# mrinmoy-iitg/SM_HPSS_MTL

Hardware: AMD Instinct MI355X
Metric: clips/sec HPSS+MTL-CNN fwd (1s@16kHz) (higher is better)
Workload: dtype f32

## Files before the change

### sm_hpss_mtl_amd/csrc/smh_model.h

```cpp
#pragma once
#include "smh_common.h"

namespace smh_tcn {

using f32x4 = __attribute__((ext_vector_type(4))) float;

constexpr int C = 32;
constexpr int SX = 36;
constexpr int kMaxHeads = 4;
constexpr int kHidden = 16;
constexpr int kMaxG = 16;
constexpr int kPS = 80;
constexpr float kNormEps = 1e-5f;
constexpr float kBnEps = 1e-3f;
constexpr int kCat = kHidden + 2;
constexpr int kCatTail = 4 * kHidden + 4 * kCat + kCat + 1;
constexpr int kBlockFloats = 24 * 2 * 64 + 8 * 2 * 64 + 32 + 32;
constexpr size_t kNetLdsLimit = smh::kLdsBytesPerCU - 4 * 1024;

struct TcnArgs {
    int N, T, F, FQ, G, GRP, n_blocks, n_dil, vec_ok;
    int D, NH, n_mt, n_classes, n_heads, out_dim, skip_heads;
    int wlds;
    unsigned long long *trace;
    int tune;
    int *status;
    int spin_limit;
    int split_last;
    int from_x0;
    int x0_shift, x0_T;
    int head_odim[kMaxHeads];
    int head_sigmoid[kMaxHeads];
    int cascade;
    int single;
    int trunk_only;
    int x0_one;
    const float *pair_X, *pair_W0, *pair_Wb;
    float *pair_trunk;
    const float *pair_WhA, *pair_hp;
    float *pair_out;
    int *pair_status;
};

struct TrainIO {
    float *acts;
    const float *drop_tcn;
    float *pre;
    float *upre;
    int acts_last_only;
};

struct HeadsArgs {
    int N, D, NH, n_classes, n_heads, out_dim;
    int head_odim[kMaxHeads], head_sigmoid[kMaxHeads];
    float lw[kMaxHeads + 1];
    size_t goff_head[kMaxHeads];
    size_t goff_c3b;
    size_t hp_off[kMaxHeads];
    int ext_losses;
    int stamps;
};
struct HeadsPlan;
int launch_heads_train(const HeadsArgs &a, const HeadsPlan &p, const float *pre, const float *y, const float *hp, const float *drop,
                       float *dpre, float *dxh, float *grad, float *bnstat, float *losses, unsigned *ticket, hipStream_t st);
int launch_cascade_heads_train(const HeadsArgs &a, const HeadsPlan &p, const float *pre, const float *y, const float *hp,
                               const float *drop, float *dpre, float *dxh, float *dr, float *grad, float *bnstat, float *losses,
                               hipStream_t st);
// ... 21 lines not shown
    int *d_map = nullptr;
    size_t nW0, nWb, nWhA, nhp;
    void *d_bf16 = nullptr;
    unsigned long long version = 1, bf16_version = 0;
    int *d_status = nullptr;
};

namespace smh_tcn {
inline size_t head_tail_floats(const smh_model *m, int h) {
    const int od = m->head_odim[h], cat = m->head_cat[h];
    return cat ? (size_t)4 * kHidden + 4 * cat + (size_t)cat * od + od : (size_t)4 * kHidden + (size_t)kHidden * od + od;
}
struct Offsets {
    size_t w0_k, w0_b;
    size_t blk0, blk_stride;
    size_t c3_k, c3_b;
    size_t head[kMaxHeads];
    size_t trunk_p = 0;
    size_t fbn = 0;
};
inline size_t trunk_floats(const smh_model_cfg &c) {
    return (size_t)c.n_feat * C + C + (size_t)c.nb_stacks * c.n_dilations * (3 * C * C + C + C * C + C);
}
__host__ __device__ inline size_t v2_block0_floats(int F) {
    return (size_t)3 * F * C + C + 3 * C * C + C + (F != C ? (size_t)F * C + C : 0);
}
constexpr size_t kV2BlockFloats = 2 * (3 * C * C + C);
inline size_t trunk_floats_v2(const smh_model_cfg &c) {
    return v2_block0_floats(c.n_feat) + (size_t)(c.nb_stacks * c.n_dilations - 1) * kV2BlockFloats;
}
Offsets offsets(const smh_model *m);
struct ForwardSwitches {
    int G = 0, skew = -1, waves = 0;
    bool has_waves = false, prefetch = true, split = true, skew16 = false;
};
ForwardSwitches read_forward_switches();
struct ForwardPlan {
    int G, GRP, units, nwaves, mode, wlds, split_last;
    size_t lds;
};
int plan_forward(const smh_model *m, int N, bool train, bool trace, const ForwardSwitches &sw, ForwardPlan *p);
void fill_args(const smh_model *m, int N, const ForwardPlan &p, TcnArgs *a);
int dense_entry_ok(const char *name, const smh_model *m, const float *d_fv, int Tc, int shift, const void *d_work, size_t work_bytes,
                   size_t need_bytes, const float *d_out, int feat_multiple, const char *short_clip_entry);
int repack(smh_model *m, hipStream_t st);
int launch_forward_bf16_train(smh_model *m, const float *d_x, int N, const TrainIO *tio, hipStream_t st);
int forward_bf16_supported(const smh_model *m);
struct ForwardOpts {
    int from_x0 = 0, x0_shift = 0, x0_T = 0;
    int trunk_only = 0;
    int x0_one = 0;
    const smh_model *pair = nullptr;
    const float *pair_x = nullptr;
    float *pair_trunk = nullptr;
    float *pair_out = nullptr;
};
int launch_forward(const smh_model *m, const float *d_x, int N, float *d_out, float *d_trunk, const TrainIO *tio,
                   hipStream_t st, const ForwardOpts &opt = {});
int launch_l0_frames(const float *fv, const float *w0, float *x0, int rows, int Tc, hipStream_t st);
int launch_fusion_dense(const smh_model *m, int N, const float *xh, const float *xp, float *out, bool train, hipStream_t st);
size_t fusion_scratch_floats(const smh_model *m, int max_batch);
int launch_fusion_train(const smh_model *m, int N, int max_batch, const float *acts_h, const float *acts_p, float *scratch,
                        float *bnstat, float *pd, float *grad, int phase, hipStream_t st);
const float *fusion_gt(const smh_model *m, int max_batch, const float *scratch, int N, int b);
int launch_fusion_trunks(const smh_model *m, const float *xh, const float *xp, int N, float *tap_h, float *tap_p, ForwardOpts fo,
                         hipStream_t st);
// ... 3 lines not shown
```

### sm_hpss_mtl_amd/csrc/smh_tcn.hip

```cpp
#include <algorithm>
#include <cmath>
#include <cstdlib>
#include <cstring>
#include <type_traits>
#include <vector>

#include "smh_model.h"
#include "smh_tcn_heads.h"

using namespace smh_tcn;

namespace {

__device__ __forceinline__ f32x4 mfma4(float a, float b, f32x4 c) {
    return __builtin_amdgcn_mfma_f32_16x16x4f32(a, b, c, 0, 0, 0);
}

__device__ __forceinline__ float quad_max(float v) {
    const unsigned u = __float_as_uint(v);
    const auto r32 = __builtin_amdgcn_permlane32_swap(u, u, false, false);
    const float a = fmaxf(__uint_as_float(r32[0]), __uint_as_float(r32[1]));
    const unsigned ua = __float_as_uint(a);
    const auto r16 = __builtin_amdgcn_permlane16_swap(ua, ua, false, false);
    return fmaxf(__uint_as_float(r16[0]), __uint_as_float(r16[1]));
// ... 389 lines not shown
            }
        } else {
            for (int i = threadIdx.x; i < nW0; i += blockDim.x) w0s[i] = W0[i];
            __syncthreads();
            for (int u = wave; u < units; u += nw) {
                const int R = 16 * u + j;
                const int Rc = min(R, GR - 1);
                const float *xr = X + ((size_t)n0 * T + Rc) * a.F + (size_t)q * a.FQ;
                f32x4 c0 = bl, c1 = bh;
                for (int s = 0; s < a.FQ; ++s) {
                    const float xv = (q * a.FQ + s < a.F) ? xr[s] : 0.f;
                    c0 = mfma4(w0s[(s * 2 + 0) * 64 + lane], xv, c0);
                    c1 = mfma4(w0s[(s * 2 + 1) * 64 + lane], xv, c1);
                }
                float *dst = xa + (size_t)R * SX + 4 * q;
                *reinterpret_cast<f32x4 *>(dst) = c0;
                *reinterpret_cast<f32x4 *>(dst + 16) = c1;
            }
        }
    }

    float *ws = lds + 2 * (size_t)(a.GRP + 1) * SX;
    auto stage = [&](int blk) {
        const char *src = reinterpret_cast<const char *>(Wb + (size_t)blk * kBlockFloats);
        char *dst = reinterpret_cast<char *>(ws + (size_t)(blk & 1) * kBlockFloats);
        constexpr int nch = kBlockFloats * 4 / 16;
        for (int i = wave; i * 64 < nch; i += nw) {
            const int c = i * 64 + lane;
            if (c < nch)
                __builtin_amdgcn_global_load_lds((const __attribute__((address_space(1))) void *)(src + (size_t)c * 16),
                                                 (__attribute__((address_space(3))) void *)(dst + i * 1024), 16, 0, 0);
        }
    };
    TileInfo ti;
    ti.n = 0;
    const bool split = MODE == kPrefetch && a.split_last && units >= 2;
#pragma unroll
    for (int i = 0; i < kMaxTiles; ++i) {
        const int u = wave + i * nw;
        const int R = 16 * u + j, Rc = min(R, GR - 1);
        ti.R[i] = R, ti.g[i] = Rc / T, ti.t[i] = Rc - ti.g[i] * T;
        if (u < units - (split ? 1 : 0)) ti.n = i + 1;
    }
    {
        const int hw0 = (units - 1) % nw, hw1 = (hw0 + 1) % nw;
        ti.hrole = split ? (wave == hw0 ? 0 : (wave == hw1 ? 1 : -1)) : -1;
        const int R = 16 * (units - 1) + j, Rc = min(R, GR - 1);
        ti.hR = R, ti.hg = Rc / T, ti.ht = Rc - ti.hg * T;
    }
    float *xch = lds + 2 * (size_t)(a.GRP + 1) * SX + 2 * (size_t)kBlockFloats;
    if (split && threadIdx.x < 2) reinterpret_cast<int *>(xch + 2 * 64 * 4)[threadIdx.x] = 0;
    if (threadIdx.x < SX) xa[(size_t)ZR * SX + threadIdx.x] = 0.f, xb[(size_t)ZR * SX + threadIdx.x] = 0.f;
    float *xin = xa, *xout = xb;
    const int nslot = a.n_blocks + 1;
    auto save_acts = [&](const float *src, int slot) {
        if constexpr (TRAIN) {
            for (int i = threadIdx.x; i < GR * (C / 4); i += blockDim.x) {
                const int R = i >> 3, c4 = (i & 7) * 4;
                const int g = R / T, t = R - g * T;
                *reinterpret_cast<f32x4 *>(tio.acts + (((size_t)(n0 + g) * nslot + slot) * T + t) * C + c4) =
                    *reinterpret_cast<const f32x4 *>(src + (size_t)R * SX + c4);
            }
        }
    };
    const float *drop0 = TRAIN && tio.drop_tcn ? tio.drop_tcn + (size_t)n0 * a.n_blocks * C : nullptr;
    const int dstride = a.n_blocks * C;
// ... 5 lines not shown
                         ub0 ? ub0 + (size_t)blk * T * C : nullptr, ustride, prefetch, lane, xch, blk + 1, a.spin_limit, status);
        float *tmp = xin;
        xin = xout;
        xout = tmp;
    };
    if (MODE != kSkew && MODE != kSkew16 && tracing && blockIdx.x < 1024 && threadIdx.x == 0) {
        a.trace[4 * (2000 + blockIdx.x)] = __builtin_amdgcn_s_memtime();
        a.trace[4 * (2000 + blockIdx.x) + 1] = __builtin_amdgcn_s_memrealtime();
    }
    static_assert(!(TRAIN && MODE == kSkew16), "the 16-wave schedule is built for inference");
    float *flagbase = ws + (MODE == kSkew16 ? (size_t)kWeightRing * kBlockFloats : 0);
    if constexpr (MODE == kSkew || MODE == kSkew16) {
        typedef __attribute__((address_space(3))) volatile int lds_vint;
        lds_vint *done = (lds_vint *)(flagbase);
        if (threadIdx.x < 64) {
            int v = threadIdx.x == 62 ? nw : 0;
            if (MODE == kSkew16 && threadIdx.x >= 56 && threadIdx.x < 60)
                v = (threadIdx.x - 56 < 2 && threadIdx.x - 56 < a.n_blocks) ? threadIdx.x - 56 : -1;
            done[threadIdx.x] = v;
        }
        auto stage_ring = [&](int blk, int w0, int nwv) {
            const char *src = reinterpret_cast<const char *>(Wb + (size_t)blk * kBlockFloats);
            char *dst = reinterpret_cast<char *>(ws + (size_t)(blk & (kWeightRing - 1)) * kBlockFloats);
            constexpr int nch = kBlockFloats * 4 / 16;
            for (int i = w0; i * 64 < nch; i += nwv) {
                const int c = i * 64 + lane;
                if (c < nch)
                    __builtin_amdgcn_global_load_lds((const __attribute__((address_space(1))) void *)(src + (size_t)c * 16),
                                                     (__attribute__((address_space(3))) void *)(dst + i * 1024), 16, 0, 0);
            }
        };
        BlockW w0, w1;
        if constexpr (MODE == kSkew) {
            load_block_lds(w0, Wb, lane, q);
        } else {
            stage_ring(0, wave, nw);
            if (a.n_blocks > 1) stage_ring(1, wave, nw);
            asm volatile("s_waitcnt vmcnt(0)" ::: "memory");
        }
        __syncthreads();
        save_acts(xin, 0);
        if constexpr (TRAIN) __syncthreads();
        if (tracing && blockIdx.x < 1024 && threadIdx.x == 0) {
            a.trace[4 * (2000 + blockIdx.x)] = __builtin_amdgcn_s_memtime();
            a.trace[4 * (2000 + blockIdx.x) + 1] = __builtin_amdgcn_s_memrealtime();
        }
        const int n_tasks = a.n_blocks * units;
        const int m_units = (65536 + units - 1) / units, m_dil = (65536 + a.n_dil - 1) / a.n_dil;
        const unsigned m_T = (unsigned)(((1ull << 32) + (unsigned)T - 1) / (unsigned)T);
        const unsigned all_tiles = units >= 32 ? ~0u : (1u << units) - 1;
        const int xb_off = (a.GRP + 1) * SX, zrow = ZR * SX + 8 * q;
        struct Ops {
            f32x4 b[3][2], r0, r1;
            bool live0, live2;
            f32x4 dm0, dm1;
            int arow, urow;
        };
        auto dil = [&](int blk) { return 1 << (blk - ((blk * m_dil) >> 16) * a.n_dil); };
        auto ld4 = [&](int i) { return *reinterpret_cast<const f32x4 *>(__builtin_assume_aligned(lds + i, 16)); };
        auto issue_ops = [&](Ops &o, int blk, int u) {
            const int d = dil(blk);
            const int base = 16 * u, R = base + j;
            int g = (int)__umulhi((unsigned)base, m_T);
            int t = base - T * g + j;
            {
                const bool wr = t >= T;
// ... 213 lines not shown
                            if (stands(have, blk - 1, all_tiles)) break;
                            if (__any(lane == 63 && have != 0)) break;
                            if (spins > a.spin_limit) {
                                if (lane == 0) done[63] = 1;
                                break;
                            }
                            __builtin_amdgcn_s_sleep(1);
                        }
                    }
                    staged = blk + 2;
                    stage_ring(staged, 0, 1);
                }
                one_task(LdsWeights{ws + (size_t)(blk & (kWeightRing - 1)) * kBlockFloats, lane, q});
            }
        }
        publish();
        xin = (a.n_blocks & 1) ? xb : xa;
        xout = (a.n_blocks & 1) ? xa : xb;
        if (tracing && blockIdx.x < 1024 && threadIdx.x == 0) {
            a.trace[4 * (2000 + blockIdx.x) + 2] = __builtin_amdgcn_s_memtime();
            a.trace[4 * (2000 + blockIdx.x) + 3] = __builtin_amdgcn_s_memrealtime();
        }
    } else if (a.wlds && MODE == kPrefetch) {
        BlockW w0, w1;
        stage(0);
        if (a.n_blocks > 1) stage(1);
        asm volatile("s_waitcnt vmcnt(0)" ::: "memory");
        __syncthreads();
        load_block_lds(w0, ws, lane, q);
        for (int blk = 0; blk < a.n_blocks; blk += 2) {
            asm volatile("s_waitcnt vmcnt(0)" ::: "memory");
            __syncthreads();
            if (blk + 2 < a.n_blocks) stage(blk + 2);
            const bool more1 = blk + 1 < a.n_blocks;
            one_block(blk, w0, WeightPrefetch{w1, ws + kBlockFloats, lane, q});
            if (!more1) break;
            asm volatile("s_waitcnt vmcnt(0)" ::: "memory");
            __syncthreads();
            if (blk + 3 < a.n_blocks) stage(blk + 3);
            one_block(blk + 1, w1, WeightPrefetch{w0, ws, lane, q});
        }
    } else {
        if (a.wlds) stage(0);
        BlockW w;
        for (int blk = 0; blk < a.n_blocks; ++blk) {
            if (a.wlds) {
                asm volatile("s_waitcnt vmcnt(0)" ::: "memory");
                __syncthreads();
                if (blk + 1 < a.n_blocks) stage(blk + 1);
                one_block(blk, w, WeightLoad{w, ws + (size_t)(blk & 1) * kBlockFloats, lane, q});
            } else {
                __syncthreads();
                load_block_lds(w, Wb + (size_t)blk * kBlockFloats, lane, q);
                one_block(blk, w, NoPrefetch());
            }
        }
    }
    if (MODE != kSkew && MODE != kSkew16 && tracing && blockIdx.x < 1024 && threadIdx.x == 0) {
        a.trace[4 * (2000 + blockIdx.x) + 2] = __builtin_amdgcn_s_memtime();
        a.trace[4 * (2000 + blockIdx.x) + 3] = __builtin_amdgcn_s_memrealtime();
    }
    __syncthreads();
    if constexpr (MODE != kSkew && MODE != kSkew16) save_acts(xin, a.n_blocks);
    if constexpr (TRAIN) __syncthreads();
    for (int i = threadIdx.x; i < GR * (C / 4); i += blockDim.x) {
        const int R = i >> 3, c4 = (i & 7) * 4;
        f32x4 v = *reinterpret_cast<const f32x4 *>(xin + (size_t)R * SX + c4);
#pragma unroll
        for (int r = 0; r < 4; ++r) v[r] = fmaxf(v[r], 0.f);
        *reinterpret_cast<f32x4 *>(xin + (size_t)R * SX + c4) = v;
        if (trunk) *reinterpret_cast<f32x4 *>(trunk + ((size_t)n0 * T + R) * C + c4) = v;
    }
    __syncthreads();

    bool gave_up = false;
    if constexpr (MODE == kSkew || MODE == kSkew16) gave_up = ((__attribute__((address_space(3))) volatile int *)(flagbase))[63] != 0;
    dense_and_heads<TRAIN>(a, xin, xout, WhA, hp, out, tio, n0, g_here);
    if (tracing && blockIdx.x < 256 && threadIdx.x == 0) a.trace[4 * 3000 + 2 * blockIdx.x + 1] = __builtin_amdgcn_s_memrealtime();
    if (gave_up) {
        __syncthreads();
        for (int i = threadIdx.x; i < (a.trunk_only ? 0 : g_here * a.out_dim); i += blockDim.x) out[(size_t)n0 * a.out_dim + i] = 0.f;
        if (threadIdx.x == 0 && status) atomicOr(status, 1);
    }
}

__global__ void repack_kernel(const float *__restrict__ flat, const int *__restrict__ map, float *__restrict__ dst, size_t n) {
    const size_t i = (size_t)blockIdx.x * blockDim.x + threadIdx.x;
    if (i < n) {
        const int m = map[i];
        dst[i] = m ? flat[m - 1] : 0.f;
    }
}

static void pack_host(const smh_model *m, const float *h, std::vector<float> &W0, std::vector<float> &Wb,
                      std::vector<float> &WhA, std::vector<float> &hp) {
    const int F = m->cfg.n_feat, FQ = m->FQ, D = m->D, NH = m->NH, ncls = m->cfg.n_classes;
    W0.assign(m->nW0, 0.f), Wb.assign(m->nWb, 0.f), WhA.assign(m->nWhA, 0.f), hp.assign(m->nhp, 0.f);
    std::vector<float> Wh((size_t)D * NH, 0.f), bhv((size_t)m->n_mt * 16, 0.f);
    const float *p = h;
    if (m->heads == SMH_HEADS_FUSION) {
        p += 2 * trunk_floats(m->cfg) + (size_t)4 * D;
    } else if (m->cfg.block_variant == 1) {
        p += trunk_floats_v2(m->cfg);
    } else {
    for (int s = 0; s < FQ; ++s)
        for (int mt = 0; mt < 2; ++mt)
            for (int lane = 0; lane < 64; ++lane) {
                const int q = lane >> 4, i = lane & 15, f = q * FQ + s;
                W0[((size_t)s * 2 + mt) * 64 + lane] = f < F ? p[(size_t)f * C + 16 * mt + i] : 0.f;
            }
// ... 103 lines not shown
}

int repack(smh_model *m, hipStream_t st) {
    m->version++;
    if (m->heads == SMH_HEADS_FUSION) {
        const size_t tf = trunk_floats(m->cfg);
        for (int b = 0; b < 2; ++b) {
            SMH_CHECK_HIP(hipMemcpyAsync(m->trunk[b]->d_flat, m->d_flat + b * tf, tf * sizeof(float), hipMemcpyDeviceToDevice, st));
            const int rc = repack(m->trunk[b], st);
            if (rc) return rc;
            const size_t k0 = (size_t)m->cfg.n_feat * C;
            SMH_CHECK_HIP(hipMemcpyAsync(m->d_w0cat + b * k0, m->d_flat + b * tf, k0 * sizeof(float), hipMemcpyDeviceToDevice, st));
        }
    }
    const size_t n = m->nW0 + m->nWb + m->nWhA + m->nhp;
    hipLaunchKernelGGL(repack_kernel, dim3((unsigned)((n + 255) / 256)), dim3(256), 0, st, m->d_flat, m->d_map, m->d_W0, n);
    return smh::launch_status("repack_kernel");
}

void fill_args(const smh_model *m, int N, const ForwardPlan &p, TcnArgs *pa) {
    TcnArgs &a = *pa;
    a.N = N, a.T = m->cfg.patch_size, a.F = m->cfg.n_feat, a.FQ = m->FQ, a.n_blocks = m->n_blocks, a.n_dil = m->cfg.n_dilations;
    a.vec_ok = (a.F % 4 == 0) && (a.FQ % 4 == 0) && (a.FQ * 4 == a.F);
    a.skip_heads = 0;
    a.trunk_only = 0;
    a.tune = 0;
    a.trace = nullptr;
    a.from_x0 = 0, a.x0_shift = 0, a.x0_T = 0, a.x0_one = 0;
    a.pair_X = a.pair_W0 = a.pair_Wb = nullptr, a.pair_trunk = nullptr;
    a.pair_WhA = a.pair_hp = nullptr, a.pair_out = nullptr, a.pair_status = nullptr;
    a.status = m->d_status, a.spin_limit = kSkewSpinLimit;
    a.D = m->D, a.NH = m->NH, a.n_mt = m->n_mt, a.n_classes = m->cfg.n_classes, a.n_heads = m->n_heads;
    a.out_dim = m->out_dim;
    for (int i = 0; i < kMaxHeads; ++i) a.head_odim[i] = m->head_odim[i], a.head_sigmoid[i] = m->head_sigmoid[i];
    a.cascade = m->heads == SMH_HEADS_CASCADED;
    a.single = m->heads == SMH_HEADS_SINGLE;
    a.G = p.G, a.GRP = p.GRP, a.wlds = p.wlds, a.split_last = p.split_last;
}

ForwardSwitches read_forward_switches() {
    const auto num = [](const char *ev, int unset) { return ev ? atoi(ev) : unset; };
    ForwardSwitches s;
    s.G = num(getenv("SMH_TCN_G"), 0);
    s.skew = num(getenv("SMH_TCN_SKEW"), -1);
    const char *waves = getenv("SMH_TCN_WAVES");
    s.has_waves = waves != nullptr, s.waves = num(waves, 0);
    s.prefetch = num(getenv("SMH_TCN_PREFETCH"), 1) != 0;
    s.split = num(getenv("SMH_TCN_SPLIT"), 1) != 0;
    s.skew16 = num(smh::lab_env("SMH_TCN_SKEW16"), 0) != 0;
    return s;
}

int plan_forward(const smh_model *m, int N, bool train, bool trace, const ForwardSwitches &sw, ForwardPlan *pp) {
    ForwardPlan &p = *pp;
    const int T = m->cfg.patch_size;
    int gmax = 272 / T;
    if (gmax < 1) gmax = 1;
    if (gmax > kMaxG) gmax = kMaxG;
    int G = (N + 255) / 256;
    if (G < 1) G = 1;
    if (G > gmax) G = gmax;
    if (sw.G >= 1 && sw.G <= gmax) G = sw.G;
    p.G = G;
    int GRP = ((G * T + 15) / 16) * 16;
    const int head_scratch = 8 * 4 * 128 + kMaxG * kPS;
    if (GRP * SX < head_scratch) GRP = (head_scratch + SX - 1) / SX;
    if (GRP * SX < m->FQ * 2 * 64) GRP = (m->FQ * 2 * 64 + SX - 1) / SX;
    GRP = ((GRP + 15) / 16) * 16;
    p.GRP = GRP;
    const size_t lds_x = sizeof(float) * 2 * (size_t)(GRP + 1) * SX, lds_w = sizeof(float) * 2 * (size_t)kBlockFloats;
    const size_t lds_xch = sizeof(float) * (2 * 64 * 4 + 4);
    p.wlds = lds_x + lds_w + lds_xch <= kNetLdsLimit ? 1 : 0;
    p.lds = lds_x + (p.wlds ? lds_w + lds_xch : 0);
    SMH_REQUIRE(p.lds <= kNetLdsLimit, "patch_size %d too long for the LDS-resident TCN", T);
    const int units = p.units = (std::min(G, N) * T + 15) / 16;
    int nwaves = 8;
    for (int w = 9; w <= 12 && !p.wlds; ++w)
        if ((units + w - 1) / w < (units + nwaves - 1) / nwaves) nwaves = w;
    if (sw.has_waves) nwaves = std::max(4, std::min(12, sw.waves));
    const bool prefetch = nwaves <= 8 && p.wlds && sw.prefetch;
    const bool skew_ok = p.wlds && units <= 32 && units >= 1 && m->n_blocks * units < 2048 && T >= 16;
    bool skew = skew_ok && units >= 12 && 8 * ((units + 7) / 8) - units >= 3 && units != 13;
// ... 18 lines not shown
    if (trace) {
        if (mode == kSkew) return b3mtl_forward_kernel<false, kSkew, true>;
        if (mode == kPrefetch) return b3mtl_forward_kernel<false, kPrefetch, true>;
        return b3mtl_forward_kernel<false, kOneSet, true>;
    }
#ifdef SMH_LAB
    if (mode == kSkew16) return b3mtl_forward_kernel<false, kSkew16, false>;
#endif
    if (mode == kSkew) return b3mtl_forward_kernel<false, kSkew, false>;
    if (mode == kPrefetch) return b3mtl_forward_kernel<false, kPrefetch, false>;
    return b3mtl_forward_kernel<false, kOneSet, false>;
}

static bool same_trunk_geometry(const smh_model *m, const smh_model *p) {
    return p->cfg.n_feat == m->cfg.n_feat && p->cfg.patch_size == m->cfg.patch_size && p->n_blocks == m->n_blocks &&
           p->cfg.n_dilations == m->cfg.n_dilations && p->nW0 == m->nW0 && p->nWb == m->nWb && p->nW0 > 0;
}
static bool same_head_geometry(const smh_model *m, const smh_model *p) {
    return p->heads == m->heads && p->cfg.n_classes == m->cfg.n_classes && p->nWhA == m->nWhA && p->nhp == m->nhp && p->out_dim == m->out_dim;
}

int launch_forward(const smh_model *m, const float *d_x, int N, float *d_out, float *d_trunk, const TrainIO *tio,
                   hipStream_t st, const ForwardOpts &opt) {
    const smh_model *pm = opt.pair;
    if (pm && opt.pair_out) {
        SMH_REQUIRE(!tio && !opt.trunk_only && d_out && opt.pair_x, "paired full forward: inference of two whole models, each to its own output");
        SMH_REQUIRE(same_trunk_geometry(m, pm) && same_head_geometry(m, pm), "paired full forward: the two models differ in geometry or head kind");
    } else if (pm) {
        SMH_REQUIRE(!tio && opt.trunk_only && d_trunk && opt.pair_x && opt.pair_trunk, "paired trunk launch: inference to the trunk taps only");
        SMH_REQUIRE(same_trunk_geometry(m, pm), "paired trunk launch: the two trunks differ in geometry");
    }
    unsigned long long *trace = g_trace ? g_trace + (g_trace_launches++ & 1) * kTraceWords : nullptr;
    ForwardPlan p;
    const int rc = plan_forward(m, N, tio != nullptr, trace != nullptr, read_forward_switches(), &p);
    if (rc) return rc;
    TcnArgs a;
    fill_args(m, N, p, &a);
    a.trace = trace;
    a.trunk_only = opt.trunk_only;
    a.from_x0 = opt.from_x0, a.x0_shift = opt.x0_shift, a.x0_T = opt.x0_T;
    a.x0_one = opt.from_x0 ? opt.x0_one : 0;
    if (const char *ev = smh::probe_env("SMH_TCN_BLOCKS")) a.n_blocks = atoi(ev);
    a.skip_heads = smh::probe_env("SMH_TCN_NOHEADS") ? 1 : 0;
    if (const char *ev = smh::probe_env("SMH_TCN_TUNE")) a.tune = atoi(ev);
    if (a.tune & 256) a.spin_limit = 1 << 10;
    if (pm) {
        a.pair_X = opt.pair_x, a.pair_W0 = pm->d_W0, a.pair_Wb = pm->d_Wb, a.pair_trunk = opt.pair_trunk;
        a.pair_status = opt.pair_out ? pm->d_status : a.status;
        if (opt.pair_out) a.pair_WhA = pm->d_WhA, a.pair_hp = pm->d_hp, a.pair_out = opt.pair_out;
    }
    const TrainIO io = tio ? *tio : TrainIO{nullptr, nullptr, nullptr, nullptr};
    return smh::launch_lds(pick_forward_kernel(tio != nullptr, p.mode, trace != nullptr), "b3mtl_forward_kernel",
                           dim3((N + p.G - 1) / p.G, pm ? 2 : 1), dim3(64 * p.nwaves), p.lds, p.lds, st, a, d_x, m->d_W0, m->d_Wb, m->d_WhA,
                           m->d_hp, d_trunk, d_out, io);
}

int dense_entry_ok(const char *name, const smh_model *m, const float *d_fv, int Tc, int shift, const void *d_work, size_t work_bytes,
                   size_t need_bytes, const float *d_out, int feat_multiple, const char *short_clip_entry) {
    SMH_REQUIRE(m && d_fv && d_work && d_out, "%s: null argument", name);
    SMH_REQUIRE((reinterpret_cast<uintptr_t>(d_work) % 16) == 0 && (reinterpret_cast<uintptr_t>(d_fv) % 16) == 0 &&
                    (reinterpret_cast<uintptr_t>(d_out) % 4) == 0,
                "%s: d_fv and d_work are read / written with 16-byte accesses and must start on 16-byte boundaries", name);
    const int W = m->cfg.patch_size, F = m->cfg.n_feat;
    if (feat_multiple == 8)
        SMH_REQUIRE(F % 8 == 0, "%s: n_feat=%d must be a multiple of 8 (two halves of whole k steps)", name, F);
    else
        SMH_REQUIRE(F % feat_multiple == 0, "%s: the per-branch n_feat=%d must be a multiple of %d (whole k steps per half)", name, F, feat_multiple);
    SMH_REQUIRE(shift >= 1 && Tc >= W, "%s: needs shift >= 1 and at least patch_size=%d frames (Tc=%d, shift=%d); "
                "shorter chunks are tiled by get_feature_patches and take %s", name, W, Tc, shift, short_clip_entry);
    SMH_REQUIRE(work_bytes >= need_bytes, "%s: workspace of %zu bytes, need %zu", name, work_bytes, need_bytes);
// ... 347 lines not shown
```

### sm_hpss_mtl_amd/csrc/smh_tcn_heads.h

```cpp
#pragma once
#include <type_traits>

#include "smh_model.h"

namespace smh_tcn {

__device__ __forceinline__ void cascaded_r(const TcnArgs &a, const float *pp, const float *bh, const float *hp, float r[2]) {
    const float *ph = hp + 2 * kCatTail;
    const float *gamma = ph, *beta = ph + 16, *mean = ph + 32, *var = ph + 48, *wo = ph + 64, *bo = wo + 2 * kHidden;
    r[0] = bo[0], r[1] = bo[1];
#pragma unroll
    for (int i = 0; i < kHidden; ++i) {
        const int o = a.n_classes + 2 * kHidden + i;
        float v = pp[o] + bh[o];
        v = (v - mean[i]) / sqrtf(var[i] + kBnEps);
        v = fmaxf(v * gamma[i] + beta[i], 0.f);
        r[0] = fmaf(v, wo[2 * i], r[0]);
        r[1] = fmaf(v, wo[2 * i + 1], r[1]);
    }
}

__device__ __forceinline__ void cascaded_head(const TcnArgs &a, const float *pp, const float *bh, const float *hp, float *orow, int h) {
    float r[2];
    cascaded_r(a, pp, bh, hp, r);
// ... 58 lines not shown
    } else if (tid >= 128 && tid < 128 + g_here) {
        const int p = tid - 128;
        float mxl = -INFINITY;
        for (int c = 0; c < a.n_classes; ++c) mxl = fmaxf(mxl, pre[p * kPS + c] + bh[c]);
        float den = 0.f;
        for (int c = 0; c < a.n_classes; ++c) den += expf(pre[p * kPS + c] + bh[c] - mxl);
        const int col = a.out_dim - a.n_classes;
        for (int c = 0; c < a.n_classes; ++c)
            out[(size_t)(n0 + p) * a.out_dim + col + c] = expf(pre[p * kPS + c] + bh[c] - mxl) / den;
    }
}

__device__ __forceinline__ void single_tail(const TcnArgs &a, const float *pre, const float *bh, float *__restrict__ out, int n0,
                                            int g_here) {
    const int p = threadIdx.x;
    if (p >= g_here) return;
    constexpr int kMaxC = 5;
    float z[kMaxC], mx = -INFINITY, den = 0.f;
#pragma unroll
    for (int c = 0; c < kMaxC; ++c) {
        z[c] = c < a.n_classes ? pre[p * kPS + c] + bh[c] : -INFINITY;
        mx = fmaxf(mx, z[c]);
    }
#pragma unroll
    for (int c = 0; c < kMaxC; ++c) {
        z[c] = c < a.n_classes ? expf(z[c] - mx) : 0.f;
        den += z[c];
    }
#pragma unroll
    for (int c = 0; c < kMaxC; ++c)
        if (c < a.n_classes) out[(size_t)(n0 + p) * a.out_dim + c] = z[c] / den;
}

template <bool TRAIN>
__device__ __forceinline__ void dense_and_heads(const TcnArgs &a, const float *xin, float *xout, const float *__restrict__ WhA,
                                                const float *__restrict__ hp, float *__restrict__ out, const TrainIO &tio,
                                                int n0, int g_here) {
    if (a.trunk_only) return;
    const int wave = threadIdx.x >> 6, lane = threadIdx.x & 63, nw = blockDim.x >> 6;
    const int T = a.T;
    const int OPL = (a.NH + 63) >> 6;
    const int ld = OPL * 64;
    constexpr int kDenseParts = 8;
    float *part = xout;
    float *pre = xout + (size_t)kDenseParts * 4 * ld;
    const int rpp = (T + kDenseParts - 1) / kDenseParts;
    auto dense_on_trunk = [&](auto opl_c) {
        constexpr int kOPL = decltype(opl_c)::value;
        for (int g0 = 0; g0 < g_here; g0 += 4) {
            const float *xg[4];
#pragma unroll
            for (int g = 0; g < 4; ++g) xg[g] = xin + (size_t)min(g0 + g, g_here - 1) * T * SX;
            for (int pt = wave; pt < kDenseParts; pt += nw) {
                const int t_lo = min(T, pt * rpp), t_hi = min(T, t_lo + rpp);
                float acc[4][kOPL];
#pragma unroll
                for (int g = 0; g < 4; ++g)
#pragma unroll
                    for (int p = 0; p < kOPL; ++p) acc[g][p] = 0.f;
                for (int t = t_lo; t < t_hi; ++t) {
                    const f32x4 *wrow = reinterpret_cast<const f32x4 *>(WhA) + (size_t)t * (C / 4) * ld + lane;
#pragma unroll 2
                    for (int c8 = 0; c8 < 4; ++c8) {
                        f32x4 wa[kOPL], wb[kOPL];
#pragma unroll
                        for (int p = 0; p < kOPL; ++p) {
                            wa[p] = wrow[(size_t)(2 * c8) * ld + 64 * p];
                            wb[p] = wrow[(size_t)(2 * c8 + 1) * ld + 64 * p];
                        }
#pragma unroll
                        for (int g = 0; g < 4; ++g) {
                            const f32x4 xa = *reinterpret_cast<const f32x4 *>(xg[g] + (size_t)t * SX + 8 * c8);
                            const f32x4 xb = *reinterpret_cast<const f32x4 *>(xg[g] + (size_t)t * SX + 8 * c8 + 4);
#pragma unroll
                            for (int c = 0; c < 4; ++c)
#pragma unroll
                                for (int p = 0; p < kOPL; ++p) {
                                    acc[g][p] = fmaf(xa[c], wa[p][c], acc[g][p]);
                                    acc[g][p] = fmaf(xb[c], wb[p][c], acc[g][p]);
                                }
                        }
                    }
                }
#pragma unroll
                for (int g = 0; g < 4; ++g)
#pragma unroll
                    for (int p = 0; p < kOPL; ++p) part[((size_t)pt * 4 + g) * ld + 64 * p + lane] = acc[g][p];
            }
            __syncthreads();
            for (int i = threadIdx.x; i < 4 * ld; i += blockDim.x) {
                const int g = i / ld, o = i - g * ld;
                if (g0 + g < g_here && o < kPS) {
                    float v = 0.f;
#pragma unroll
                    for (int pt = 0; pt < kDenseParts; ++pt) v += part[((size_t)pt * 4 + g) * ld + o];
                    pre[(g0 + g) * kPS + o] = v;
                }
            }
            __syncthreads();
        }
    };
    if (!a.skip_heads) {
        if (OPL == 1) dense_on_trunk(std::integral_constant<int, 1>{});
        else dense_on_trunk(std::integral_constant<int, 2>{});
    }
    const float *bh = WhA + (size_t)a.D * ld;
    if constexpr (TRAIN) {
        for (int i = threadIdx.x; i < g_here * kPS; i += blockDim.x) {
            const int p = i / kPS, o = i - p * kPS;
            tio.pre[(size_t)(n0 + p) * kPS + o] = o < a.NH ? pre[p * kPS + o] + bh[o] : 0.f;
        }
        return;
    }
    if (a.single) single_tail(a, pre, bh, out, n0, g_here);
    else heads_tail(a, pre, bh, hp, out, n0, g_here);
}

}
```

### sm_hpss_mtl_amd/csrc/smh_tcn_v2.hip

```cpp
#include <algorithm>
#include <cstdlib>

#include "smh_model.h"
#include "smh_tcn_heads.h"

using namespace smh_tcn;

namespace {

__device__ __forceinline__ f32x4 mfma4(float a, float b, f32x4 c) { return __builtin_amdgcn_mfma_f32_16x16x4f32(a, b, c, 0, 0, 0); }

struct ConvW {
    float w[24][2];
    f32x4 blo, bhi;
};

__device__ __forceinline__ void load_conv(ConvW &cw, const float *__restrict__ k, const float *__restrict__ b, int q, int i) {
#pragma unroll
    for (int tap = 0; tap < 3; ++tap)
#pragma unroll
        for (int s8 = 0; s8 < 8; ++s8) {
            const float *p = k + ((size_t)tap * C + 8 * q + s8) * C + i;
            cw.w[tap * 8 + s8][0] = p[0];
            cw.w[tap * 8 + s8][1] = p[16];
// ... 120 lines not shown
            conv_tile(cw, xa, Rc, t, d, T, ZR, q, y0, y1);
#pragma unroll
            for (int r = 0; r < 4; ++r) y0[r] = fmaxf(y0[r], 0.f), y1[r] = fmaxf(y1[r], 0.f);
            float *dst = ya + (size_t)R * SX + 4 * q;
            *reinterpret_cast<f32x4 *>(dst) = y0;
            *reinterpret_cast<f32x4 *>(dst + 16) = y1;
        }
        load_conv(cw, k1, k1 + 3 * C * C, q, j);
        __syncthreads();
        for (int u = wave; u < units; u += nw) {
            const int R = 16 * u + j, Rc = min(R, GR - 1);
            const int t = Rc % T;
            f32x4 y0, y1;
            conv_tile(cw, ya, Rc, t, d, T, ZR, q, y0, y1);
            float *xr = xa + (size_t)Rc * SX + 4 * q;
            f32x4 s0 = *reinterpret_cast<const f32x4 *>(xr), s1 = *reinterpret_cast<const f32x4 *>(xr + 16);
#pragma unroll
            for (int r = 0; r < 4; ++r) {
                s0[r] = fmaxf(s0[r] + fmaxf(y0[r], 0.f), 0.f);
                s1[r] = fmaxf(s1[r] + fmaxf(y1[r], 0.f), 0.f);
            }
            float *dst = xa + (size_t)R * SX + 4 * q;
            *reinterpret_cast<f32x4 *>(dst) = s0;
            *reinterpret_cast<f32x4 *>(dst + 16) = s1;
        }
    }
    __syncthreads();
    if (trunk)
        for (int i = threadIdx.x; i < GR * (C / 4); i += blockDim.x) {
            const int R = i >> 3, c4 = (i & 7) * 4;
            *reinterpret_cast<f32x4 *>(trunk + ((size_t)n0 * T + R) * C + c4) = *reinterpret_cast<const f32x4 *>(xa + (size_t)R * SX + c4);
        }
    TrainIO none{nullptr, nullptr, nullptr, nullptr};
    dense_and_heads<false>(a, xa, ya, WhA, hp, out, none, n0, g_here);
}

}

namespace smh_tcn {

int launch_forward_v2(const smh_model *m, const float *d_x, int N, float *d_out, float *d_trunk, hipStream_t st) {
    ForwardPlan p;
    const int rc = plan_forward(m, N, false, false, read_forward_switches(), &p);
    if (rc) return rc;
    TcnArgs a;
    fill_args(m, N, p, &a);
    const size_t lds = sizeof(float) * 2 * (size_t)(a.GRP + 1) * SX;
    SMH_REQUIRE(lds <= kNetLdsLimit, "patch_size %d too long for the LDS-resident TCN", a.T);
    const dim3 grid((N + a.G - 1) / a.G), block(512);
    SMH_CHECK_HIP(hipFuncSetAttribute((const void *)b3mtl_forward_v2_kernel, hipFuncAttributeMaxDynamicSharedMemorySize, (int)lds));
    hipLaunchKernelGGL(b3mtl_forward_v2_kernel, grid, block, lds, st, a, d_x, (const float *)m->d_flat, (const float *)m->d_WhA,
                       (const float *)m->d_hp, d_trunk, d_out);
    return smh::launch_status("b3mtl_forward_v2_kernel");
}

}
```

### sm_hpss_mtl_amd/csrc/smh_train.hip

```cpp
#include <cmath>
#include <cstdlib>
#include <cstring>
#include <vector>

#include <type_traits>

#include "smh_model.h"
#include "smh_train_bwd.h"
#include "smh_train_plan.h"
#include "smh_wave.h"

using namespace smh_tcn;

namespace {

constexpr float kKerasEps = 1e-7f;
constexpr float kBnMomentum = 0.99f;
constexpr float kL2 = 0.01f;
static_assert(Dims::C == C && Dims::SX == SX && Dims::PS == kPS && Dims::Hidden == kHidden && Dims::MaxHeads == kMaxHeads &&
                  Dims::LdsPerCU == (size_t)smh::kLdsBytesPerCU && Dims::NetLdsLimit == kNetLdsLimit,
              "smh_train_plan.h: Dims");

using smh_tcn::HeadsArgs;

// ... 1121 lines not shown
    if (e == hipSuccess)
        e = hipMalloc((void **)&t->d_upre, (size_t)max_batch * m->n_blocks * m->cfg.patch_size * C * (fusion ? 2 : 1) * sizeof(float));
    if (e == hipSuccess && fusion) e = hipMalloc((void **)&t->d_fusion, fusion_scratch_floats(m, max_batch) * sizeof(float));
    if (e == hipSuccess) e = hipMalloc((void **)&t->d_l2part, (kMaxHeads * kL2Chunks + 1) * sizeof(double));
    if (e == hipSuccess) e = hipMemset(t->d_l2part, 0, (kMaxHeads * kL2Chunks + 1) * sizeof(double));
    if (e == hipSuccess) e = hipMalloc((void **)&t->d_segs, segs.size() * sizeof(Segment));
    if (e == hipSuccess) e = hipMemcpy(t->d_segs, segs.data(), segs.size() * sizeof(Segment), hipMemcpyHostToDevice);
    if (e == hipSuccess) e = hipMemset(t->d_vel, 0, m->n_params * sizeof(float));
    if (e == hipSuccess) e = hipMemset(t->d_s2, 0, m->n_params * sizeof(float));
    if (e == hipSuccess) e = hipMemset(t->d_grad, 0, (m->n_params + t->bn_floats) * sizeof(float));
    if (e != hipSuccess) {
        smh_trainer_destroy(t);
        return smh::set_error(SMH_E_HIP, "smh_trainer_create: device allocation failed: %s", hipGetErrorString(e));
    }
    *out = t;
    return SMH_OK;
}

extern "C" void smh_trainer_destroy(smh_trainer *t) {
    if (!t) return;
    for (float *p : {t->d_acts, t->d_pre, t->d_dpre, t->d_dxh, t->d_grad, t->d_vel, t->d_s2, t->d_sumsq, t->d_scratch_out, t->d_upre})
        (void)hipFree(p);
    (void)hipFree(t->d_segs);
    (void)hipFree(t->d_l2part);
    (void)hipFree(t->d_gq);
    (void)hipFree(t->d_bwd_pack);
    (void)hipFree(t->d_gt);
    (void)hipFree(t->d_dr);
    (void)hipFree(t->d_fusion);
    delete t;
}

extern "C" float *smh_trainer_grad_ptr(smh_trainer *t) { return t ? t->d_grad : nullptr; }

static int det_finalize(smh_trainer *t, hipStream_t st) {
    if (!t->d_gq) return SMH_OK;
    const size_t n = t->m->n_params;
    hipLaunchKernelGGL(det_finalize_kernel, dim3((unsigned)((n + 255) / 256)), dim3(256), 0, st, t->d_gq, t->d_grad, n);
    return smh::launch_status("det_finalize_kernel");
}

extern "C" int smh_trainer_set_deterministic(smh_trainer *t, int on, void *stream) {
    SMH_REQUIRE(t, "smh_trainer_set_deterministic: null trainer");
    hipStream_t st = (hipStream_t)stream;
    if (on && !t->d_gq) {
        SMH_CHECK_HIP(hipMalloc((void **)&t->d_gq, t->m->n_params * sizeof(unsigned long long)));
        SMH_CHECK_HIP(hipMemsetAsync(t->d_gq, 0, t->m->n_params * sizeof(unsigned long long), st));
    } else if (!on && t->d_gq) {
        SMH_CHECK_HIP(hipStreamSynchronize(st));
        (void)hipFree(t->d_gq);
        t->d_gq = nullptr;
    }
    return SMH_OK;
}

extern "C" int smh_model_check_train_dtype(const smh_model *m, int dtype) {
    SMH_REQUIRE(m, "smh_model_check_train_dtype: null model");
    SMH_REQUIRE(dtype == 0 || dtype == 1, "smh_trainer_set_dtype: dtype must be 0 (f32) or 1 (split bf16 operands)");
    SMH_REQUIRE(dtype == 0 || m->heads == SMH_HEADS_MTL,
                "smh_trainer_set_dtype: the split-bf16 training step has the B3_MTL heads only; a cascaded, intermediate-fusion or "
                "single-task model trains in f32 (dtype 0)");
    return dtype == 0 ? SMH_OK : forward_bf16_supported(m);
}

extern "C" int smh_trainer_set_dtype(smh_trainer *t, int dtype) {
    SMH_REQUIRE(t, "smh_trainer_set_dtype: null trainer");
// ... 259 lines not shown
```

Baseline: 2.753 million.

## Stream dense-head weights through buffer loads and pre-stage exit weights into LDS

Adds a new dense_stream path for the flatten-dense layer. It streams WhA rows through buffer loads with a register ring and uses DPP quad FMAs. While the last TCN block computes, it issues async global-to-LDS copies of the head bias, the head params and the first dense weight rows into the freed weight ring, so the tail reads them from LDS. This aims to hide the global-load latency of the dense/heads epilogue behind trunk compute, at the cost of more code paths, extra register pressure and an added vmcnt wait before the heads.

```diff
diff --git a/sm_hpss_mtl_amd/csrc/smh_model.h b/sm_hpss_mtl_amd/csrc/smh_model.h
--- a/sm_hpss_mtl_amd/csrc/smh_model.h
+++ b/sm_hpss_mtl_amd/csrc/smh_model.h
@@ -33,6 +33,8 @@
     int head_sigmoid[kMaxHeads];
     int cascade;
     int single;
+    int nhp;
+    int exit_level;
     int trunk_only;
     int x0_one;
     const float *pair_X, *pair_W0, *pair_Wb;
@@ -120,6 +122,7 @@
 Offsets offsets(const smh_model *m);
 struct ForwardSwitches {
     int G = 0, skew = -1, waves = 0;
+    int exit_level = 3;
     bool has_waves = false, prefetch = true, split = true, skew16 = false;
 };
 ForwardSwitches read_forward_switches();
diff --git a/sm_hpss_mtl_amd/csrc/smh_tcn.hip b/sm_hpss_mtl_amd/csrc/smh_tcn.hip
--- a/sm_hpss_mtl_amd/csrc/smh_tcn.hip
+++ b/sm_hpss_mtl_amd/csrc/smh_tcn.hip
@@ -445,6 +445,11 @@
                                                  (__attribute__((address_space(3))) void *)(dst + i * 1024), 16, 0, 0);
         }
     };
+    const int last_blk = a.n_blocks - 1;
+    float *exit_dst = MODE == kSkew ? ws + 128 : ws + (size_t)((last_blk & 1) ^ (MODE == kOneSet ? 1 : 0)) * kBlockFloats;
+    const int exit_cap = MODE == kSkew ? 2 * kBlockFloats - 128 : kBlockFloats;
+    const bool exit_staged = !TRAIN && MODE != kSkew16 && a.exit_level >= 2 && a.wlds && a.n_blocks >= 1 && !a.trunk_only &&
+                             !a.skip_heads && exit_stage_fits(a, exit_cap);
     TileInfo ti;
     ti.n = 0;
     const bool split = MODE == kPrefetch && a.split_last && units >= 2;
@@ -516,6 +521,7 @@
         };
         BlockW w0, w1;
         if constexpr (MODE == kSkew) {
+            if (exit_staged && wave == nw - 1) exit_stage_issue(a, WhA, hp, exit_dst, exit_cap, 0, 1);
             load_block_lds(w0, Wb, lane, q);
         } else {
             stage_ring(0, wave, nw);
@@ -795,12 +801,14 @@
             asm volatile("s_waitcnt vmcnt(0)" ::: "memory");
             __syncthreads();
             if (blk + 2 < a.n_blocks) stage(blk + 2);
+            else if (blk == last_blk && exit_staged) exit_stage_issue(a, WhA, hp, exit_dst, exit_cap, wave, nw);
             const bool more1 = blk + 1 < a.n_blocks;
             one_block(blk, w0, WeightPrefetch{w1, ws + kBlockFloats, lane, q});
             if (!more1) break;
             asm volatile("s_waitcnt vmcnt(0)" ::: "memory");
             __syncthreads();
             if (blk + 3 < a.n_blocks) stage(blk + 3);
+            else if (blk + 1 == last_blk && exit_staged) exit_stage_issue(a, WhA, hp, exit_dst, exit_cap, wave, nw);
             one_block(blk + 1, w1, WeightPrefetch{w0, ws, lane, q});
         }
     } else {
@@ -811,6 +819,7 @@
                 asm volatile("s_waitcnt vmcnt(0)" ::: "memory");
                 __syncthreads();
                 if (blk + 1 < a.n_blocks) stage(blk + 1);
+                else if (exit_staged) exit_stage_issue(a, WhA, hp, exit_dst, exit_cap, wave, nw);
                 one_block(blk, w, WeightLoad{w, ws + (size_t)(blk & 1) * kBlockFloats, lane, q});
             } else {
                 __syncthreads();
@@ -823,6 +832,7 @@
         a.trace[4 * (2000 + blockIdx.x) + 2] = __builtin_amdgcn_s_memtime();
         a.trace[4 * (2000 + blockIdx.x) + 3] = __builtin_amdgcn_s_memrealtime();
     }
+    if (exit_staged) asm volatile("s_waitcnt vmcnt(0)" ::: "memory");
     __syncthreads();
     if constexpr (MODE != kSkew && MODE != kSkew16) save_acts(xin, a.n_blocks);
     if constexpr (TRAIN) __syncthreads();
@@ -838,7 +848,7 @@
 
     bool gave_up = false;
     if constexpr (MODE == kSkew || MODE == kSkew16) gave_up = ((__attribute__((address_space(3))) volatile int *)(flagbase))[63] != 0;
-    dense_and_heads<TRAIN>(a, xin, xout, WhA, hp, out, tio, n0, g_here);
+    dense_and_heads<TRAIN, MODE == kOneSet || TRAIN>(a, xin, xout, WhA, hp, out, tio, n0, g_here, exit_staged ? exit_dst : nullptr, exit_cap);
     if (tracing && blockIdx.x < 256 && threadIdx.x == 0) a.trace[4 * 3000 + 2 * blockIdx.x + 1] = __builtin_amdgcn_s_memrealtime();
     if (gave_up) {
         __syncthreads();
@@ -1008,6 +1018,7 @@
     a.status = m->d_status, a.spin_limit = kSkewSpinLimit;
     a.D = m->D, a.NH = m->NH, a.n_mt = m->n_mt, a.n_classes = m->cfg.n_classes, a.n_heads = m->n_heads;
     a.out_dim = m->out_dim;
+    a.nhp = (int)m->nhp, a.exit_level = 0;
     for (int i = 0; i < kMaxHeads; ++i) a.head_odim[i] = m->head_odim[i], a.head_sigmoid[i] = m->head_sigmoid[i];
     a.cascade = m->heads == SMH_HEADS_CASCADED;
     a.single = m->heads == SMH_HEADS_SINGLE;
@@ -1024,6 +1035,7 @@
     s.prefetch = num(getenv("SMH_TCN_PREFETCH"), 1) != 0;
     s.split = num(getenv("SMH_TCN_SPLIT"), 1) != 0;
     s.skew16 = num(smh::lab_env("SMH_TCN_SKEW16"), 0) != 0;
+    s.exit_level = std::max(0, std::min(3, num(getenv("SMH_TCN_EXIT"), 3)));
     return s;
 }
 
@@ -1108,10 +1120,12 @@
     }
     unsigned long long *trace = g_trace ? g_trace + (g_trace_launches++ & 1) * kTraceWords : nullptr;
     ForwardPlan p;
-    const int rc = plan_forward(m, N, tio != nullptr, trace != nullptr, read_forward_switches(), &p);
+    const ForwardSwitches sw = read_forward_switches();
+    const int rc = plan_forward(m, N, tio != nullptr, trace != nullptr, sw, &p);
     if (rc) return rc;
     TcnArgs a;
     fill_args(m, N, p, &a);
+    a.exit_level = sw.exit_level;
     a.trace = trace;
     a.trunk_only = opt.trunk_only;
     a.from_x0 = opt.from_x0, a.x0_shift = opt.x0_shift, a.x0_T = opt.x0_T;
diff --git a/sm_hpss_mtl_amd/csrc/smh_tcn_heads.h b/sm_hpss_mtl_amd/csrc/smh_tcn_heads.h
--- a/sm_hpss_mtl_amd/csrc/smh_tcn_heads.h
+++ b/sm_hpss_mtl_amd/csrc/smh_tcn_heads.h
@@ -114,16 +114,69 @@
         if (c < a.n_classes) out[(size_t)(n0 + p) * a.out_dim + c] = z[c] / den;
 }
 
-template <bool TRAIN>
+__device__ __forceinline__ f32x4 as_f32x4(__attribute__((ext_vector_type(4))) unsigned v) { return __builtin_bit_cast(f32x4, v); }
+constexpr int kOutOfRange = 0x40000000;
+using f32x2 = __attribute__((ext_vector_type(2))) float;
+template <int J>
+__device__ __forceinline__ float quad_fma(float x, float w, float acc) {
+    static_assert(J >= 0 && J < 4, "a lane of the quad");
+    if constexpr (J == 0) asm("v_fmac_f32_dpp %0, %1, %2 quad_perm:[0,0,0,0] row_mask:0xf bank_mask:0xf bound_ctrl:1" : "+v"(acc) : "v"(x), "v"(w));
+    if constexpr (J == 1) asm("v_fmac_f32_dpp %0, %1, %2 quad_perm:[1,1,1,1] row_mask:0xf bank_mask:0xf bound_ctrl:1" : "+v"(acc) : "v"(x), "v"(w));
+    if constexpr (J == 2) asm("v_fmac_f32_dpp %0, %1, %2 quad_perm:[2,2,2,2] row_mask:0xf bank_mask:0xf bound_ctrl:1" : "+v"(acc) : "v"(x), "v"(w));
+    if constexpr (J == 3) asm("v_fmac_f32_dpp %0, %1, %2 quad_perm:[3,3,3,3] row_mask:0xf bank_mask:0xf bound_ctrl:1" : "+v"(acc) : "v"(x), "v"(w));
+    return acc;
+}
+
+constexpr int kDenseParts = 8;
+
+struct ExitLayout {
+    int bh_off, rows_off, R;
+};
+__device__ __forceinline__ ExitLayout exit_layout(const TcnArgs &a, int ld, int cap) {
+    ExitLayout l;
+    l.bh_off = (a.nhp + 3) & ~3;
+    l.rows_off = l.bh_off + ((a.NH + 3) & ~3);
+    l.R = min(C / 4, max(0, cap - l.rows_off) / (4 * ld * kDenseParts));
+    return l;
+}
+__device__ __forceinline__ bool exit_stage_fits(const TcnArgs &a, int cap) {
+    return ((a.nhp + 3) & ~3) + ((a.NH + 3) & ~3) <= cap;
+}
+__device__ __forceinline__ void exit_stage_issue(const TcnArgs &a, const float *__restrict__ WhA, const float *__restrict__ hp,
+                                                 float *dst, int cap, int first, int stride) {
+    const int lane = threadIdx.x & 63;
+    const int kb_row = (a.NH + 63) >> 6, ld = 64 * kb_row;
+    const ExitLayout l = exit_layout(a, ld, cap);
+    const int nhc = (a.nhp + 63) >> 6, nbc = kb_row, nrow = kDenseParts * l.R * kb_row;
+    const int rpp = (a.T + kDenseParts - 1) / kDenseParts;
+    typedef const __attribute__((address_space(1))) void *gptr;
+    typedef __attribute__((address_space(3))) void *lptr;
+    for (int i = first; i < nhc + nbc + nrow; i += stride) {
+        if (i < nhc + nbc) {
+            const bool is_hp = i < nhc;
+            const int c = is_hp ? i : i - nhc, n = is_hp ? a.nhp : a.NH;
+            const float *src = is_hp ? hp : WhA + (size_t)a.D * ld;
+            if (64 * c + lane < n)
+                __builtin_amdgcn_global_load_lds((gptr)(src + 64 * c + lane), (lptr)(dst + (is_hp ? 0 : l.bh_off) + 64 * c), 4, 0, 0);
+        } else {
+            const int k = i - nhc - nbc, row = k / kb_row, h = k - row * kb_row;
+            const int pt = row / l.R, r = row - pt * l.R, t_lo = pt * rpp;
+            if (t_lo < a.T)
+                __builtin_amdgcn_global_load_lds((gptr)(WhA + ((size_t)t_lo * (C / 4) + r) * ld * 4 + 256 * h + 4 * lane),
+                                                 (lptr)(dst + l.rows_off + (size_t)row * ld * 4 + 256 * h), 16, 0, 0);
+        }
+    }
+}
+
+template <bool TRAIN, bool LEAN = false>
 __device__ __forceinline__ void dense_and_heads(const TcnArgs &a, const float *xin, float *xout, const float *__restrict__ WhA,
                                                 const float *__restrict__ hp, float *__restrict__ out, const TrainIO &tio,
-                                                int n0, int g_here) {
+                                                int n0, int g_here, const float *stg = nullptr, int stg_cap = 0) {
     if (a.trunk_only) return;
     const int wave = threadIdx.x >> 6, lane = threadIdx.x & 63, nw = blockDim.x >> 6;
     const int T = a.T;
     const int OPL = (a.NH + 63) >> 6;
     const int ld = OPL * 64;
-    constexpr int kDenseParts = 8;
     float *part = xout;
     float *pre = xout + (size_t)kDenseParts * 4 * ld;
     const int rpp = (T + kDenseParts - 1) / kDenseParts;
@@ -182,9 +235,115 @@
             __syncthreads();
         }
     };
+    const int level = a.exit_level;
+    const ExitLayout sl = stg ? exit_layout(a, ld, stg_cap) : ExitLayout{0, 0, 0};
+    auto dense_stream = [&](auto opl_c) {
+        constexpr int kOPL = decltype(opl_c)::value;
+        constexpr int NST = (LEAN ? 4 : 8) / kOPL;
+        const int nh_lim = level >= 3 ? a.NH : 64 * kOPL;
+        for (int g0 = 0; g0 < g_here; g0 += 4) {
+            const float *xg[4];
+#pragma unroll
+            for (int g = 0; g < 4; ++g) xg[g] = xin + (size_t)min(g0 + g, g_here - 1) * T * SX;
+            for (int pt = __builtin_amdgcn_readfirstlane(wave); pt < kDenseParts; pt += nw) {
+                const int t_lo = min(T, pt * rpp), t_hi = min(T, t_lo + rpp);
+                float acc[4][kOPL];
+#pragma unroll
+                for (int g = 0; g < 4; ++g)
+#pragma unroll
+                    for (int p = 0; p < kOPL; ++p) acc[g][p] = 0.f;
+                if (t_lo < t_hi) {
+                    const int n_steps = 4 * (t_hi - t_lo);
+                    const int row_bytes = ld * 16;
+                    const auto rsrc = __builtin_amdgcn_make_buffer_rsrc(const_cast<float *>(WhA) + (size_t)t_lo * (C / 4) * ld * 4, 0,
+                                                                        2 * n_steps * row_bytes, 0x00020000);
+                    const f32x4 *srow = reinterpret_cast<const f32x4 *>(stg + sl.rows_off) + (size_t)pt * sl.R * ld + lane;
+                    int voff[kOPL];
+#pragma unroll
+                    for (int p = 0; p < kOPL; ++p) voff[p] = lane + 64 * p < nh_lim ? 16 * (lane + 64 * p) : kOutOfRange;
+                    f32x4 wa[NST][kOPL], wb[NST][kOPL];
+                    auto request = [&](int i, int s, auto lds_c) {
+#pragma unroll
+                        for (int p = 0; p < kOPL; ++p)
+#pragma unroll
+                            for (int h = 0; h < 2; ++h) {
+                                const int r = 2 * s + h;
+                                f32x4 &w = h ? wb[i][p] : wa[i][p];
+                                if constexpr (decltype(lds_c)::value) {
+                                    const bool staged = r < sl.R;
+                                    const f32x4 ws = srow[(size_t)min(r, sl.R - 1) * ld + 64 * p];
+                                    const f32x4 wg = as_f32x4(__builtin_amdgcn_raw_buffer_load_b128(
+                                        rsrc, voff[p] + r * row_bytes + (staged ? kOutOfRange : 0), 0, 0));
+                                    w = staged ? ws : wg;
+                                } else {
+                                    w = as_f32x4(__builtin_amdgcn_raw_buffer_load_b128(rsrc, voff[p] + r * row_bytes, 0, 0));
+                                }
+                            }
+                    };
+                    auto products = [&](int i, int s) {
+                        const int t = t_lo + (s >> 2), c8 = s & 3;
+#pragma unroll
+                        for (int g = 0; g < 4; ++g) {
+                            const f32x2 xv = *reinterpret_cast<const f32x2 *>(xg[g] + (size_t)t * SX + 8 * c8 + 2 * (lane & 3));
+                            auto channel = [&](auto cc) {
+                                constexpr int c = decltype(cc)::value;
+#pragma unroll
+                                for (int p = 0; p < kOPL; ++p) {
+                                    acc[g][p] = quad_fma<c / 2>(xv[c & 1], wa[i][p][c], acc[g][p]);
+                                    acc[g][p] = quad_fma<2 + c / 2>(xv[c & 1], wb[i][p][c], acc[g][p]);
+                                }
+                            };
+                            channel(std::integral_constant<int, 0>{}), channel(std::integral_constant<int, 1>{});
+                            channel(std::integral_constant<int, 2>{}), channel(std::integral_constant<int, 3>{});
+                        }
+                    };
+                    if (sl.R > 0) {
+#pragma unroll
+                        for (int i = 0; i < NST; ++i) {
+                            if (i < 4) request(i, i, std::true_type{});
+                            else request(i, i, std::false_type{});
+                        }
+                    } else {
+#pragma unroll
+                        for (int i = 0; i < NST; ++i) request(i, i, std::false_type{});
+                    }
+                    for (int s0 = 0; s0 < n_steps; s0 += NST) {
+#pragma unroll
+                        for (int i = 0; i < NST; ++i) {
+                            if (NST == 8 && i == 4 && s0 + 4 >= n_steps) break;
+                            products(i, s0 + i), request(i, s0 + i + NST, std::false_type{});
+                            if constexpr (LEAN) __builtin_amdgcn_sched_barrier(0);
+                        }
+                    }
+                }
+#pragma unroll
+                for (int g = 0; g < 4; ++g)
+#pragma unroll
+                    for (int p = 0; p < kOPL; ++p) part[((size_t)pt * 4 + g) * ld + 64 * p + lane] = acc[g][p];
+            }
+            __syncthreads();
+            for (int i = threadIdx.x; i < 4 * ld; i += blockDim.x) {
+                const int g = i / ld, o = i - g * ld;
+                if (g0 + g < g_here && o < kPS) {
+                    float v = 0.f;
+                    if (level < 3 || o < a.NH) {
+#pragma unroll
+                        for (int pt = 0; pt < kDenseParts; ++pt) v += part[((size_t)pt * 4 + g) * ld + o];
+                    }
+                    pre[(g0 + g) * kPS + o] = v;
+                }
+            }
+            __syncthreads();
+        }
+    };
     if (!a.skip_heads) {
-        if (OPL == 1) dense_on_trunk(std::integral_constant<int, 1>{});
-        else dense_on_trunk(std::integral_constant<int, 2>{});
+        if (level == 0) {
+            if (OPL == 1) dense_on_trunk(std::integral_constant<int, 1>{});
+            else dense_on_trunk(std::integral_constant<int, 2>{});
+        } else {
+            if (OPL == 1) dense_stream(std::integral_constant<int, 1>{});
+            else dense_stream(std::integral_constant<int, 2>{});
+        }
     }
     const float *bh = WhA + (size_t)a.D * ld;
     if constexpr (TRAIN) {
@@ -194,6 +353,11 @@
         }
         return;
     }
+    if (stg) {
+        if (a.single) single_tail(a, pre, stg + sl.bh_off, out, n0, g_here);
+        else heads_tail(a, pre, stg + sl.bh_off, stg, out, n0, g_here);
+        return;
+    }
     if (a.single) single_tail(a, pre, bh, out, n0, g_here);
     else heads_tail(a, pre, bh, hp, out, n0, g_here);
 }
diff --git a/sm_hpss_mtl_amd/csrc/smh_tcn_v2.hip b/sm_hpss_mtl_amd/csrc/smh_tcn_v2.hip
--- a/sm_hpss_mtl_amd/csrc/smh_tcn_v2.hip
+++ b/sm_hpss_mtl_amd/csrc/smh_tcn_v2.hip
@@ -176,7 +176,7 @@
             *reinterpret_cast<f32x4 *>(trunk + ((size_t)n0 * T + R) * C + c4) = *reinterpret_cast<const f32x4 *>(xa + (size_t)R * SX + c4);
         }
     TrainIO none{nullptr, nullptr, nullptr, nullptr};
-    dense_and_heads<false>(a, xa, ya, WhA, hp, out, none, n0, g_here);
+    dense_and_heads<false, true>(a, xa, ya, WhA, hp, out, none, n0, g_here);
 }
 
 }
@@ -185,10 +185,12 @@
 
 int launch_forward_v2(const smh_model *m, const float *d_x, int N, float *d_out, float *d_trunk, hipStream_t st) {
     ForwardPlan p;
-    const int rc = plan_forward(m, N, false, false, read_forward_switches(), &p);
+    const ForwardSwitches sw = read_forward_switches();
+    const int rc = plan_forward(m, N, false, false, sw, &p);
     if (rc) return rc;
     TcnArgs a;
     fill_args(m, N, p, &a);
+    a.exit_level = sw.exit_level;
     const size_t lds = sizeof(float) * 2 * (size_t)(a.GRP + 1) * SX;
     SMH_REQUIRE(lds <= kNetLdsLimit, "patch_size %d too long for the LDS-resident TCN", a.T);
     const dim3 grid((N + a.G - 1) / a.G), block(512);
diff --git a/sm_hpss_mtl_amd/csrc/smh_train.hip b/sm_hpss_mtl_amd/csrc/smh_train.hip
--- a/sm_hpss_mtl_amd/csrc/smh_train.hip
+++ b/sm_hpss_mtl_amd/csrc/smh_train.hip
@@ -1177,6 +1177,7 @@
 }
 
 extern "C" float *smh_trainer_grad_ptr(smh_trainer *t) { return t ? t->d_grad : nullptr; }
+extern "C" const float *smh_internal_trainer_pre(const smh_trainer *t) { return t ? t->d_pre : nullptr; }
 
 static int det_finalize(smh_trainer *t, hipStream_t st) {
     if (!t->d_gq) return SMH_OK;
```

New measurement: 2.701 million. 1.9% lower.
